# NomaDamas/AutoRAG-Research

Measured on AMD Instinct MI355X. Metric: queries/sec, higher is better.
Workload: dtype f32

## Files before the change

### autorag_research_amd/csrc/dev_common.h

```cpp
#pragma once
#include <hip/hip_runtime.h>
#include <stdint.h>

namespace mi355 {

constexpr int kWave = 64;
constexpr int kQBlockMax = 1024;
constexpr int kKMax = 1024;
constexpr int kCandCap = 2048;
constexpr int kCandCapWide = 4096;
constexpr int kSortMax = 4096;
constexpr int kIrrCap = 1024;
constexpr uint64_t kKeyNaN = 0xFFFFFFFFFFFFFFFFull;

constexpr int kStOverflow = 1;
constexpr int kStIrregular = 2;

struct QueryState {
    float* qn;
    uint16_t* qhat;
    float* thr;
    int* cnt;
    int* best_n;
    uint64_t* best_key;
// ... 362 lines not shown
                    stage_commit(tile, p2, lane);
                    if (k0 + 5 * kStageCols < d) issue(p2, k0 + 5 * kStageCols);
                    acc = chain_piece(tile, lane, qv + k0 + 2 * kStageCols, min(kStageCols, d - k0 - 2 * kStageCols), acc);
                }
            }
        }
    } else {
        for (int k0 = 0; k0 < d; k0 += kStageCols) {
            stage_rows(tile, my_row, k0, d, lane);
            acc = chain_piece(tile, lane, qv + k0, min(kStageCols, d - k0), acc);
        }
    }
    return acc;
}

__device__ __forceinline__ float chain_piece16(const float* tile, int lane, const float* qv, int kn_words, float acc) {
    const float* t = tile + lane * kStageLd;
    for (int w = 0; w + 4 <= kn_words; w += 4) {
        const uint4 tv = *(const uint4*)(t + w);
        const float4 qa = *(const float4*)(qv + 2 * w), qb = *(const float4*)(qv + 2 * w + 4);
        acc = __builtin_fmaf(__uint_as_float(tv.x << 16), qa.x, acc);
        acc = __builtin_fmaf(__uint_as_float(tv.x & 0xFFFF0000u), qa.y, acc);
        acc = __builtin_fmaf(__uint_as_float(tv.y << 16), qa.z, acc);
        acc = __builtin_fmaf(__uint_as_float(tv.y & 0xFFFF0000u), qa.w, acc);
        acc = __builtin_fmaf(__uint_as_float(tv.z << 16), qb.x, acc);
        acc = __builtin_fmaf(__uint_as_float(tv.z & 0xFFFF0000u), qb.y, acc);
        acc = __builtin_fmaf(__uint_as_float(tv.w << 16), qb.z, acc);
        acc = __builtin_fmaf(__uint_as_float(tv.w & 0xFFFF0000u), qb.w, acc);
    }
    return acc;
// ... 23 lines not shown
```

### autorag_research_amd/csrc/index.h

```cpp
#pragma once
#include <climits>
#include <hip/hip_runtime.h>

#include <algorithm>
#include <cmath>
#include <cstdio>
#include <cstring>
#include <mutex>
#include <string>
#include <vector>

#include "dev_common.h"
#include "mi355dr.h"

namespace mi355 {
struct EventPair {
    hipEvent_t a, b;
    int big;
};
struct MultiVecStore;
struct Pending {
    bool active = false;
    hipEvent_t done = nullptr;
    int* status_host = nullptr;
// ... 48 lines not shown

    int path = 0;
    int screen_dtype = 0;
    int retry_level = 0;
    int i8_backoff = 0, i8_probation = 0;
    int i8_demoted_k = INT_MAX;
    double i8_min_budget = 0.25;
    float* retry_q[3] = {nullptr, nullptr, nullptr};
    double* retry_dist[3] = {nullptr, nullptr, nullptr};
    int64_t* retry_rows[3] = {nullptr, nullptr, nullptr};
    int* retry_map[3] = {nullptr, nullptr, nullptr};
    mi355::Pending pend[mi355::kPendingRing];
    mi355::Pending sub_pend[4];
    int64_t seq_next = 0, seq_done = 0;
    int k_now = 10;
    int maxsim_coop = -1;
    int maxsim_persistent = 0;
    int maxsim_wg = -1;
    int maxsim_tighten = 1;
    int maxsim_aligned = 1;
    int maxsim_wg_min = 8;
    int maxsim_wg_pipe = 1;
    int maxsim_pack8 = -1;
    int maxsim_wg_bps = 4;
    int maxsim_pass_groups = 4;
    int maxsim_screen = 1;
    int64_t row_offset = 0;
    int round_a = 0;
    int screen_rq = 1;
    int screen_stream = 1;
    int prefilter16 = 0;
    int profile = 0;
    int starter = 1;
    int prune_companion = 1;
    int scan_dma = 1;
    int defer_round_b = 1;
    int chunk0_set = 0;
    int64_t chunk0_rows = 1024;
    int64_t chunk_growth = 3;
    int chunk_growth_set = 0;
    int64_t small_chunk_rows = 16384;
    int cap = mi355::kCandCap;
    int cap_set = 0;
    int prune_wide = 1;
    int screen_flush_sync = 1, screen_flush_lanes = 48, screen_flush_alone = 40;
    int wide_inflation_x10 = 100;
    int flush_mask_now = -1;
    int chunk_taper_x100 = 0;
    int64_t starter_rows_wide = 65536;

    int64_t s_screen_launches = 0, s_screen_ns = 0, s_screen_rows = 0, s_fallback_queries = 0, s_chunks = 0,
            s_passes = 0, s_candidates = 0, s_rescored = 0, s_starters = 0;
    int64_t s_big_launches = 0, s_big_ns = 0, s_big_rows = 0;
    int screen_rq_split_tests = 1;
    int64_t debug_park = 0;
    float* park_thr = nullptr;
    int screen_drift = 3;
    int* rq_progress = nullptr;
    int rq_epoch = 0;
// ... 63 lines not shown
```

### autorag_research_amd/csrc/k_prune_wide.h

```cpp
#pragma once
#include <type_traits>

#include "k_select.h"

namespace mi355 {

constexpr int kWideEntries = 4096;
constexpr int kWideKeep = 512;
constexpr int kWideList = 1024;
constexpr int kWideKMin = 33, kWideKMax = 128;
constexpr int kWideSortWhole = 256;

__host__ __device__ inline size_t prune_wide_lds_bytes(int d, int waves) {
    return (size_t)kWideKeep * 12 + (size_t)waves * kStageFloats * sizeof(float) + (size_t)kWideList * 4 +
           prune_qs_floats(d) * 4;
}

__device__ __forceinline__ float f32_from_order_key(uint32_t k) {
    return __uint_as_float((k & 0x80000000u) ? (k & 0x7FFFFFFFu) : ~k);
}

template <int WAVES, int PER>
__global__ __launch_bounds__(WAVES * kWave) void k_prune_wide(PruneArgs a) {
    constexpr int T = WAVES * kWave;
    static_assert(T * PER == kWideEntries && (PER == 32 || PER == 64), "entries");
    typedef std::conditional_t<PER == 64, unsigned long long, uint32_t> amask_t;
    constexpr int KS = kWideKeep / T;
    extern __shared__ __attribute__((aligned(16))) char smem[];
    uint64_t* SK = (uint64_t*)smem;
    int32_t* SR = (int32_t*)(smem + (size_t)kWideKeep * 8);
    float* tiles = (float*)(smem + (size_t)kWideKeep * 12);
    uint64_t* K2 = (uint64_t*)tiles;
    int32_t* R2 = (int32_t*)((char*)tiles + (size_t)kWideKeep * 8);
    int32_t* RL = (int32_t*)((char*)tiles + (size_t)WAVES * kStageFloats * sizeof(float));
    float* qs = (float*)((char*)RL + (size_t)kWideList * 4);
    int* scal = (int*)(qs + prune_qs_floats(a.d) - 16);
    const int q = a.qlist ? a.qlist[blockIdx.x] : blockIdx.x;
    const int tid = threadIdx.x;
    const int lane = tid & 63;
    const int wave = __builtin_amdgcn_readfirstlane(tid >> 6);
    const int raw_cnt = a.st.cnt[q];
    const int n_best = a.st.best_n[q];
    if (raw_cnt == 0) return;
    if (raw_cnt > a.cap || raw_cnt > kWideEntries) {
        if (tid == 0) {
            a.st.status[q] |= kStOverflow;
            a.st.cnt[q] = 0;
            a.st.carry[q] = 0;
        }
        return;
    }
    const int n_new = raw_cnt;
    const int32_t* crow = a.cand_row + (int64_t)q * a.cap;
    const float* cval = a.cand_val + (int64_t)q * a.cap;
    uint64_t* bkey = a.st.best_key + (int64_t)q * kKMax;
    int32_t* brow = a.st.best_row + (int64_t)q * kKMax;
    const float nq = a.st.qn[q];
    const float inv_qn = 1.0f / sqrtf(nq);
    const float E = a.st.E[q];
    if (tid == 0) {
        a.stat[2 * q] += (unsigned long long)(n_new - a.st.carry[q]);
        scal[4] = 0;
    }

    int par = 0;
    auto wg_sum = [&](int v) __attribute__((always_inline)) -> int {
        if constexpr (WAVES == 1) return v;
        if (lane == 0) scal[par * WAVES + wave] = v;
        __syncthreads();
        int c = 0;
#pragma unroll
        for (int w = 0; w < WAVES; ++w) c += scal[par * WAVES + w];
        par ^= 1;
        return __builtin_amdgcn_readfirstlane(c);
    };
    auto wg_scan = [&](int v, int& before) __attribute__((always_inline)) -> int {
        if constexpr (WAVES == 1) {
// ... 6 lines not shown
#pragma unroll
        for (int w = 0; w < WAVES; ++w) {
            const int x = scal[par * WAVES + w];
            c += x;
            if (w < wave) b += x;
        }
        par ^= 1;
        before = __builtin_amdgcn_readfirstlane(b);
        return __builtin_amdgcn_readfirstlane(c);
    };
    auto mbcnt = [&](unsigned long long bal) __attribute__((always_inline)) -> int {
        return (int)__builtin_amdgcn_mbcnt_hi((unsigned)(bal >> 32), __builtin_amdgcn_mbcnt_lo((unsigned)bal, 0));
    };

    uint32_t key[PER];
    int32_t rowv[PER];
    amask_t in_a = 0;
    load_candidate_keys<PER, T, true>(key, cval, crow, a.flag8, n_new, tid, rowv);
    for (int k = tid; k < a.d; k += T) qs[k] = a.q[(int64_t)q * a.d + k];
    auto count_ge = [&](uint32_t x) __attribute__((always_inline)) -> int {
        int c = 0;
#pragma unroll
        for (int j = 0; j < PER; ++j) {
            if (j * T >= n_new) break;
            c += __builtin_popcountll(__builtin_amdgcn_ballot_w64(key[j] >= x));
        }
        return wg_sum(c);
    };
    const int n_cand = count_ge(1u);

    auto list_rows = [&](auto&& want, int off, int room, bool mark) __attribute__((always_inline)) -> int {
        int c = 0;
#pragma unroll
        for (int j = 0; j < PER; ++j) {
            if (j * T >= n_new) break;
            c += __builtin_popcountll(__builtin_amdgcn_ballot_w64(want(j)));
        }
        int n = 0;
        const int tot = wg_scan(c, n);
#pragma unroll
        for (int j = 0; j < PER; ++j) {
            if (j * T >= n_new) break;
            const bool w = want(j);
            const unsigned long long bal = __builtin_amdgcn_ballot_w64(w);
            const int pos = n + mbcnt(bal) - off;
            if (w && pos >= 0 && pos < room) {
                RL[pos] = rowv[j];
                if (mark) in_a |= (amask_t)1 << j;
            }
            n += __builtin_popcountll(bal);
        }
        return tot;
    };

    float* tile = tiles + (size_t)wave * kStageFloats;
    auto exact_kth_image = [&](uint32_t (&sk)[KS], int n, int kth, bool with_nan) __attribute__((always_inline)) -> uint32_t {
#pragma unroll
        for (int j = 0; j < KS; ++j) {
            const int e = j * T + tid;
            uint32_t kk = 0;
            if (e < n) {
                const uint64_t k64 = SK[e];
                if (k64 != kKeyNaN) kk = f32_order_key(sim_of_dist(a.metric, key_to_dist(k64)));
                else if (with_nan) kk = 1u;
            }
            sk[j] = kk;
        }
        uint32_t x = 0;
        for (int b = 31; b >= 0; --b) {
            const uint32_t t = x | (1u << b);
// ... 36 lines not shown
            for (int i = tid; i < n; i += T) {
                K2[i] = SK[i];
                R2[i] = SR[i];
            }
        }
        const int np = next_pow2(max(n_sel, 1));
        for (int i = n_sel + tid; i < np; i += T) {
            K2[i] = kKeyNaN;
            R2[i] = 0x7FFFFFFF;
        }
        __syncthreads();
        bitonic_asc_key_row(K2, R2, np);
        return n_sel;
    };

    const int wantA = min(n_cand, min(2 * kWave, max(a.k, a.round_a > 0 ? a.round_a : max(32, 2 * a.k))));
    int nA = 0;
    if (wantA > 0) {
        uint32_t x = 0;
        for (int b = 31; b >= 12; --b) {
            const uint32_t t = x | (1u << b);
            if (count_ge(t) >= wantA) x = t;
        }
        if (x == 0) x = 1u;
        constexpr int kAMax = 2 * kWave;
        nA = min(kAMax, list_rows([&](int j) { return key[j] >= x; }, 0, kAMax, true));
        __syncthreads();
        for (int base = 0; base < nA; base += T) {
            const int e = base + tid;
            const bool live = e < nA;
            const int32_t row = live ? RL[e] : -1;
            const float* rp = live ? a.rows + (int64_t)row * a.d : nullptr;
            if (base + wave * kWave < nA) {
                const float acc = staged_dot(tile, rp, qs, a.d, lane);
                if (live) {
                    SK[n_best + e] = dist_to_key(distance_from(a.metric, acc, nq, a.nrm2[row]));
                    SR[n_best + e] = row;
                }
            }
        }
    }
    for (int i = tid; i < n_best; i += T) {
        SK[i] = bkey[i];
        SR[i] = brow[i];
    }
    __syncthreads();
    const int n1 = n_best + nA;
    int n_sel = select_sort(n1);
    int carried = 0, nB_rescored = 0;
    if (n_cand > nA && !a.thr_only) {
        float cut = -__builtin_inff();
        uint32_t keep_x = 0;
        if (n1 >= a.k && K2[a.k - 1] != kKeyNaN) {
            const float kth = sim_of_dist(a.metric, key_to_dist(K2[a.k - 1]));
            const float ku = a.metric == 0 ? kth : kth * inv_qn;
            cut = ku - fabsf(ku) * (a.metric == 0 ? 0.0f : 4e-6f) - E * 1.001f - 2e-6f * a.cscale;
            keep_x = f32_order_key(kth);
        }
        const uint32_t xB = cut == -__builtin_inff() ? 1u : f32_order_key(cut);
        auto wantB = [&](int j) { return key[j] >= xB && key[j] != 0 && !((in_a >> j) & (amask_t)1); };
        if (a.defer_b && cut != -__builtin_inff()) {
            int32_t* crow_w = a.cand_row + (int64_t)q * a.cap;
            float* cval_w = a.cand_val + (int64_t)q * a.cap;
            int c = 0;
#pragma unroll
            for (int j = 0; j < PER; ++j) {
                if (j * T >= n_new) break;
                c += __builtin_popcountll(__builtin_amdgcn_ballot_w64(wantB(j)));
            }
            int pos0 = 0;
            carried = wg_scan(c, pos0);
#pragma unroll
            for (int j = 0; j < PER; ++j) {
                if (j * T >= n_new) break;
                const bool w = wantB(j);
                const unsigned long long bal = __builtin_amdgcn_ballot_w64(w);
                const int pos = pos0 + mbcnt(bal);
                if (w) {
                    crow_w[pos] = rowv[j];
                    cval_w[pos] = f32_from_order_key(key[j]);
                }
                pos0 += __builtin_popcountll(bal);
            }
        } else {
            const int n_keepA = min(a.k, n_sel);
            for (int i = tid; i < n_keepA; i += T) {
                SK[i] = K2[i];
                SR[i] = R2[i];
            }
            if (tid == 0) scal[4] = n_keepA;
            int totB = 0;
            for (int off = 0; off == 0 || off < totB; off += kWideList) {
                totB = list_rows(wantB, off, kWideList, false);
                __syncthreads();
                const int m = min(kWideList, totB - off);
                for (int base = 0; base < m; base += T) {
                    const int e = base + tid;
                    const bool live = e < m;
                    const int32_t row = live ? RL[e] : -1;
                    const float* rp = live ? a.rows + (int64_t)row * a.d : nullptr;
                    if (base + wave * kWave < m) {
                        const float acc = staged_dot(tile, rp, qs, a.d, lane);
                        uint64_t k64 = kKeyNaN;
                        bool pass = false;
                        if (live) {
                            k64 = dist_to_key(distance_from(a.metric, acc, nq, a.nrm2[row]));
                            pass = keep_x == 0 ||
                                   (k64 != kKeyNaN && f32_order_key(sim_of_dist(a.metric, key_to_dist(k64))) >= keep_x);
                        }
                        const unsigned long long bal = __builtin_amdgcn_ballot_w64(pass);
                        int at = 0;
                        if (lane == 0 && bal != 0) at = atomicAdd(&scal[4], __builtin_popcountll(bal));
                        at = __shfl(at, 0, kWave) + mbcnt(bal);
                        if (pass) {
                            SK[at] = k64;
                            SR[at] = row;
                        }
                    }
                    __syncthreads();
                    const int fill = __builtin_amdgcn_readfirstlane(scal[4]);
                    if (fill + T > kWideKeep) {
                        const int ns = select_sort(fill);
                        const int nk = min(a.k, ns);
                        for (int i = tid; i < nk; i += T) {
                            SK[i] = K2[i];
                            SR[i] = R2[i];
                        }
                        if (nk >= a.k && K2[a.k - 1] != kKeyNaN)
                            keep_x = max(keep_x, f32_order_key(sim_of_dist(a.metric, key_to_dist(K2[a.k - 1]))));
                        __syncthreads();
                        if (tid == 0) scal[4] = nk;
                        __syncthreads();
                    }
                }
                nB_rescored += m;
            }
            n_sel = select_sort(__builtin_amdgcn_readfirstlane(scal[4]));
        }
    }
    if (tid == 0) a.stat[2 * q + 1] += (unsigned long long)(nA + nB_rescored);
    const int n_keep = min(a.k, n_sel);
    if (!a.thr_only)
        for (int i = tid; i < n_keep; i += T) {
            bkey[i] = K2[i];
            brow[i] = R2[i];
        }
    if (tid == 0) {
        if (!a.thr_only) a.st.best_n[q] = n_keep;
        a.st.cnt[q] = carried;
        a.st.carry[q] = carried;
        if (n_keep >= a.k) {
            const uint64_t wk = K2[a.k - 1];
// ... 11 lines not shown
```

### autorag_research_amd/csrc/k_select.h

```cpp
#pragma once
#include "dev_common.h"

namespace mi355 {

struct PruneArgs {
    const float* rows;
    const float* nrm2;
    const float* q;
    QueryState st;
    int32_t* cand_row;
    float* cand_val;
    const int* qlist;
    unsigned long long* stat;
    int cap, d, k, metric;
    int exact;
    const uint8_t* flag8;
    float cscale;
    const uint16_t* shadow16;
    int dpad;
    int round_a;
    int* skip_list;
    int skip_parity;
    int thr_only;
    int one_wave_only;
    int defer_b;
};

__device__ __forceinline__ float unit_sim(int metric, double dist, float inv_qn) {
    return metric == 0 ? (float)(1.0 - dist) : (float)(-dist) * inv_qn;
}
__device__ __forceinline__ float screen_threshold(int metric, double dist_k, float E, float nq) {
    if (metric == 0) return float_below((float)((1.0 - dist_k) - (double)E));
    const double u = -dist_k / sqrt((double)nq);
    return float_below((float)(u - fabs(u) * 4e-6 - (double)E));
}

constexpr int kPruneSmallThreads = 64, kPruneSmallSort = 1024;
constexpr int kPruneBigThreads = 256, kPruneBigSort = kSortMax;

__host__ __device__ inline size_t prune_qs_floats(int d) { return ((size_t)d + 3) / 4 * 4 + 16; }
__host__ __device__ inline size_t prune_lds_bytes(int d, int threads, int sortmax, int dpad16) {
    size_t x = (size_t)(threads / kWave) * kStageFloats * sizeof(float);
    size_t lf = (size_t)sortmax * sizeof(float);
    if (lf > x) x = lf;
    return (size_t)sortmax * 8 + (size_t)sortmax * 4 + x + (size_t)sortmax * 4 + prune_qs_floats(d) * 4 + (size_t)dpad16 * 4;
}

template <int PER, int T, bool ROWS = false>
__device__ __forceinline__ void load_candidate_keys(uint32_t (&key)[PER], const float* __restrict__ cval,
                                                    const int32_t* __restrict__ crow, const uint8_t* __restrict__ flag8,
                                                    int n_new, int tid, int32_t* rows_out = nullptr) {
    float v[PER];
    int32_t r[PER];
// ... 96 lines not shown
            a.skip_list[2 + a.skip_parity * kQBlockMax + i] = q;
        }
    };
    if (raw_cnt > a.cap) {
        if (SORT < kPruneBigSort) {
            leave_for_general();
            return;
        }
        if (tid == 0) {
            a.st.status[q] |= kStOverflow;
            a.st.cnt[q] = 0;
        }
        return;
    }
    if (n_best + raw_cnt > SORT) {
        if (SORT < kPruneBigSort) leave_for_general();
        return;
    }
    const int n_new = raw_cnt;
    const int32_t* crow = a.cand_row + (int64_t)q * a.cap;
    const float* cval = a.cand_val + (int64_t)q * a.cap;
    uint64_t* bkey = a.st.best_key + (int64_t)q * kKMax;
    int32_t* brow = a.st.best_row + (int64_t)q * kKMax;
    const float nq = a.st.qn[q];
    const float inv_qn = 1.0f / sqrtf(nq);
    const float E = a.st.E[q];
    if (tid == 0) {
        a.stat[2 * q] += (unsigned long long)(n_new - a.st.carry[q]);
        a.st.carry[q] = 0;
    }

// ... 416 lines not shown
```

### autorag_research_amd/csrc/mi355dr.hip

```cpp
#include "index.h"
#include "k_prep.h"
#include "k_scan.h"
#include "k_screen.h"
#include "k_screen256c.h"
#include "k_screen_rq.h"

#define MI355_RQ_FORMS(X) X(1) X(2) X(3) X(4) X(5) X(6)
inline bool screen_rq_has(int ksteps) { return ksteps >= 1 && ksteps <= 6; }
#include "k_screen_stream.h"
#include "k_select.h"
#include "k_prune_wide.h"

using namespace mi355;

namespace {
std::mutex g_err_mu;
std::string g_err;
}

namespace mi355 {
int fail(mi355dr_index* idx, int code, const std::string& msg) {
    if (idx) idx->err = msg;
    else {
        std::lock_guard<std::mutex> g(g_err_mu);
// ... 93 lines not shown
    HIPCHECK(idx, hipMalloc(&idx->out_dist_dev, B * kKMax * sizeof(double)));
    HIPCHECK(idx, hipMalloc(&idx->out_rows_dev, B * kKMax * sizeof(int64_t)));
    HIPCHECK(idx, hipMalloc(&idx->prune_skip, (2 + 2 * B) * sizeof(int)));
    HIPCHECK(idx, hipMalloc(&idx->stat_dev, 2 * B * sizeof(unsigned long long)));
    HIPCHECK(idx, hipMemsetAsync(idx->stat_dev, 0, 2 * B * sizeof(unsigned long long), idx->stream));
    if (prune_lds_bytes(idx->dim, kPruneBigThreads, kPruneBigSort, 0) > 160 * 1024 || scan_lds_bytes(idx->dim, 1) > 160 * 1024)
        return fail(idx, MI355DR_E_UNSUPPORTED, "dim too large for the select kernels' LDS budget");
    HIPCHECK(idx, hipFuncSetAttribute((const void*)k_prune<kPruneBigThreads, kPruneBigSort>,
                                      hipFuncAttributeMaxDynamicSharedMemorySize,
                                      (int)prune_lds_bytes(idx->dim, kPruneBigThreads, kPruneBigSort, 0)));
    HIPCHECK(idx, hipFuncSetAttribute((const void*)k_prune<kPruneSmallThreads, kPruneSmallSort>,
                                      hipFuncAttributeMaxDynamicSharedMemorySize,
                                      (int)prune_lds_bytes(idx->dim, kPruneSmallThreads, kPruneSmallSort, idx->dpad)));
    HIPCHECK(idx, hipFuncSetAttribute((const void*)k_prune_wide<2, 32>, hipFuncAttributeMaxDynamicSharedMemorySize,
                                      (int)prune_wide_lds_bytes(idx->dim, 2)));
    {
        int per = kScanQ;
        while (per > 1 && scan_lds_bytes(idx->dim, per) > 150 * 1024) per >>= 1;
        HIPCHECK(idx, hipFuncSetAttribute((const void*)k_scan, hipFuncAttributeMaxDynamicSharedMemorySize,
                                          (int)scan_lds_bytes(idx->dim, per)));
    }
    HIPCHECK(idx, hipFuncSetAttribute((const void*)k_scan32, hipFuncAttributeMaxDynamicSharedMemorySize, kScan32Lds));
    HIPCHECK(idx, hipFuncSetAttribute((const void*)k_screen<false>, hipFuncAttributeMaxDynamicSharedMemorySize, kScreenLds));
    HIPCHECK(idx, hipFuncSetAttribute((const void*)k_screen<true>, hipFuncAttributeMaxDynamicSharedMemorySize, kScreenLds));
    {
        const int stream_lds = kStreamQueryBytesMax + kStreamStages * kStreamStageBytes;
        HIPCHECK(idx, hipFuncSetAttribute((const void*)k_screen_stream<false, 32>, hipFuncAttributeMaxDynamicSharedMemorySize, stream_lds));
        HIPCHECK(idx, hipFuncSetAttribute((const void*)k_screen_stream<true, 32>, hipFuncAttributeMaxDynamicSharedMemorySize, stream_lds));
        HIPCHECK(idx, hipFuncSetAttribute((const void*)k_screen_stream<false, 64>, hipFuncAttributeMaxDynamicSharedMemorySize, stream_lds));
        HIPCHECK(idx, hipFuncSetAttribute((const void*)k_screen_stream<true, 64>, hipFuncAttributeMaxDynamicSharedMemorySize, stream_lds));
// ... 39 lines not shown
        float ms = 0.f;
        if (hipEventElapsedTime(&ms, p.a, p.b) == hipSuccess) {
            idx->s_screen_ns += (int64_t)(ms * 1e6);
            if (p.big) idx->s_big_ns += (int64_t)(ms * 1e6);
        }
        idx->ev_pool.push_back(p);
    }
    idx->ev_pending.swap(keep);
}

constexpr double kInflationBf16 = 5.0, kInflationI8 = 16.0;
constexpr double kSmallBlockBudget = 1.6;
constexpr double kInflationI8Wide = 10.0, kInflationBf16Wide = 4.0;
inline bool wide_ok(const mi355dr_index* idx, int k) { return idx->prune_wide && k >= kWideKMin && k <= kWideKMax; }
inline bool wide_now(const mi355dr_index* idx) { return wide_ok(idx, idx->k_now) && idx->path != MI355DR_PATH_SCAN; }
inline int cap_now(const mi355dr_index* idx) { return !idx->cap_set && wide_now(idx) ? kCandCapWide : idx->cap; }
inline double growth_budget(const mi355dr_index* idx, int k, bool i8) {
    if (wide_ok(idx, k) && idx->path != MI355DR_PATH_SCAN) {
        const int room = std::min(kWideEntries, idx->cap_set ? idx->cap : kCandCapWide);
        return 0.75 * room / ((double)k * (i8 ? idx->wide_inflation_x10 / 10.0 : kInflationBf16Wide)) - 1.0;
    }
    const int room = k < kPruneSmallSort / 2 ? kPruneSmallSort - k : idx->cap;
    return 0.6 * std::min(room, idx->cap) / ((double)k * (i8 ? kInflationI8 : kInflationBf16));
}

inline bool i8_available(const mi355dr_index* idx) { return idx->irr8_n <= kIrrCap; }
inline bool use_i8(const mi355dr_index* idx) {
    if (idx->retry_level > 0) return false;
    if (idx->screen_dtype == MI355DR_SCREEN_I8) return true;
    return idx->screen_dtype == MI355DR_SCREEN_AUTO && i8_available(idx) && idx->k_now < idx->i8_demoted_k &&
           growth_budget(idx, idx->k_now, true) >= idx->i8_min_budget;
}

int launch_prune(mi355dr_index* idx, hipStream_t s, int nblocks, const int* qlist, int k, int exact, bool thr_only = false,
                 bool one_wave_only = false, bool defer_b = false) {
    PruneArgs pa{};
    pa.thr_only = thr_only ? 1 : 0;
    pa.one_wave_only = one_wave_only ? 1 : 0;
    pa.defer_b = defer_b && idx->defer_round_b ? 1 : 0;
    pa.rows = idx->rows;
    pa.nrm2 = idx->nrm2;
    pa.q = idx->qdev;
    pa.st = idx->st;
    pa.cand_row = idx->cand_row;
    pa.cand_val = idx->cand_val;
    pa.qlist = qlist;
    pa.stat = idx->stat_dev;
    pa.cap = cap_now(idx);
    pa.d = idx->dim;
    pa.k = k;
    pa.metric = idx->metric;
    pa.exact = exact;
    pa.flag8 = (use_i8(idx) && idx->irr8_n > 0) ? idx->flag8 : nullptr;
    pa.cscale = idx->metric == MI355DR_METRIC_IP ? idx->cmax : 1.0f;
    pa.shadow16 = (use_i8(idx) && idx->metric == 0 && !exact && idx->prefilter16) ? idx->shadow : nullptr;
    pa.dpad = idx->dpad;
    pa.round_a = idx->round_a;
    if (!exact && wide_now(idx)) {
        pa.shadow16 = nullptr;
        hipLaunchKernelGGL((k_prune_wide<2, 32>), dim3(nblocks), dim3(2 * kWave), prune_wide_lds_bytes(idx->dim, 2), s, pa);
        HIPCHECK(idx, hipGetLastError());
        return MI355DR_OK;
    }
    const bool list_mode = qlist == nullptr;
    pa.skip_list = list_mode ? idx->prune_skip : nullptr;
    pa.skip_parity = list_mode ? (idx->prune_parity ^= 1) : 0;
    hipLaunchKernelGGL((k_prune<kPruneSmallThreads, kPruneSmallSort>), dim3(nblocks), dim3(kPruneSmallThreads),
                       prune_lds_bytes(idx->dim, kPruneSmallThreads, kPruneSmallSort, pa.shadow16 ? idx->dpad : 0), s, pa);
    HIPCHECK(idx, hipGetLastError());
    if (one_wave_only) return MI355DR_OK;
    hipLaunchKernelGGL((k_prune<kPruneBigThreads, kPruneBigSort>), dim3(list_mode ? std::min(nblocks, 64) : nblocks),
                       dim3(kPruneBigThreads), prune_lds_bytes(idx->dim, kPruneBigThreads, kPruneBigSort, 0), s, pa);
    HIPCHECK(idx, hipGetLastError());
    return MI355DR_OK;
}
// ... 146 lines not shown
            const int64_t len = end - prev;
            if (len >= 2 * round_rows) end = std::min<int64_t>(n, prev + (len + round_rows / 2) / round_rows * round_rows);
        }
        if (end <= prev) continue;
        p.ends.push_back(end);
        prev = end;
        if (end >= n) break;
    }
    if (p.ends.empty() || p.ends.back() < n) p.ends.push_back(n);
    return p;
}

inline int starter_count(const PassPlan& p) { return (int)((p.sample + kSlabRows - 1) / kSlabRows); }

PassPlan make_plan(const mi355dr_index* idx, int B, int k) {
    double growth = std::max(0.25, std::min((double)idx->chunk_growth, growth_budget(idx, k, use_i8(idx))));
    if (B <= 64 && idx->retry_level == 0 && idx->chunk_growth_set == 0)
        growth = std::max(growth, std::min(8.0, growth_budget(idx, k, use_i8(idx)) * kSmallBlockBudget));
    if (idx->retry_level == 1) growth = std::max(0.25, growth * 0.5);
    if (idx->retry_level >= 2) growth = 0.25;
    return plan_pass(idx, B, k, growth);
}

int run_screen(mi355dr_index* idx, hipStream_t s, int B, int k, const PassPlan& plan) {
    int64_t kept_all_below = 0;
    const bool i8 = use_i8(idx);
    const int side_n = i8 ? idx->irr8_n : idx->irr_n;
    constexpr int kSideMerge = 32;
    bool side_done = false;
    const bool lean = plan.sample > 0 && idx->prune_companion == 0;
    auto timed = [&](bool big, int64_t rows, auto&& launch) -> int {
// ... 66 lines not shown
    st.thr_key[q] = kKeyNaN;
    st.thr_row[q] = 0x7FFFFFFF;
    st.status[q] &= ~kStOverflow;
}

int scan_range(mi355dr_index* idx, hipStream_t s, int off, int nq, int k, int64_t r0, int64_t r1) {
    ScanArgs sa{};
    sa.rows = idx->rows;
    sa.nrm2 = idx->nrm2;
    sa.q = idx->qdev;
    sa.st = idx->st;
    sa.cand_row = idx->cand_row;
    sa.cand_val = idx->cand_val;
    sa.qlist = idx->qlist_dev + off;
    sa.nq = nq;
    sa.cap = cap_now(idx);
    sa.d = idx->dim;
    sa.metric = idx->metric;
    sa.row0 = r0;
    sa.row1 = r1;
    const int64_t grid = (r1 - r0 + kScanThreads - 1) / kScanThreads;
    if (idx->dim % kScan32PieceCols == 0 && idx->scan_dma)
        hipLaunchKernelGGL(k_scan32, dim3((unsigned)grid), dim3(kScanThreads), kScan32Lds, s, sa, idx->n);
    else
        hipLaunchKernelGGL(k_scan, dim3((unsigned)grid), dim3(kScanThreads), scan_lds_bytes(idx->dim, nq), s, sa);
    HIPCHECK(idx, hipGetLastError());
    return launch_prune(idx, s, nq, idx->qlist_dev + off, k, 1);
}

int run_scan(mi355dr_index* idx, hipStream_t s, const std::vector<int>& qs, int k) {
    if (qs.empty()) return MI355DR_OK;
    HIPCHECK(idx, hipMemcpyAsync(idx->qlist_dev, qs.data(), qs.size() * sizeof(int), hipMemcpyHostToDevice, s));
    const int nq_all = (int)qs.size();
    hipLaunchKernelGGL(k_reset_queries, dim3((nq_all + 255) / 256), dim3(256), 0, s, idx->st, idx->qlist_dev, nq_all);
    HIPCHECK(idx, hipGetLastError());
    const int per = kScanQ;
    for (int off = 0; off < nq_all; off += per) {
        const int nq = std::min(per, nq_all - off);
        int64_t done = 0;
        const int cap = cap_now(idx);
        int64_t chunk = std::min<int64_t>(idx->chunk0_rows, cap);
        while (done < idx->n) {
            const int64_t end = std::min<int64_t>(idx->n, done + chunk);
            CHECK(scan_range(idx, s, off, nq, k, done, end));
            if (end - done > cap) {
                HIPCHECK(idx, hipMemcpyAsync(idx->status_host, idx->st.status, kQBlockMax * sizeof(int),
                                             hipMemcpyDeviceToHost, s));
                HIPCHECK(idx, hipStreamSynchronize(s));
                std::vector<int> redo;
                for (int j = 0; j < nq; ++j)
                    if (idx->status_host[qs[off + j]] & kStOverflow) redo.push_back(qs[off + j]);
                if (!redo.empty()) {
                    const int roff = kQBlockMax;
                    HIPCHECK(idx, hipMemcpyAsync(idx->qlist_dev + roff, redo.data(), redo.size() * sizeof(int),
                                                 hipMemcpyHostToDevice, s));
// ... 24 lines not shown
        orow[(int64_t)map[j] * k + i] = sr[(int64_t)j * k + i];
    }
}

int pending_alloc(mi355dr_index* idx, Pending& p) {
    if (!p.status_host) HIPCHECK(idx, hipHostMalloc(&p.status_host, (kQBlockMax + 1) * sizeof(int)));
    if (!p.done) HIPCHECK(idx, hipEventCreateWithFlags(&p.done, hipEventDisableTiming));
    return MI355DR_OK;
}

int enqueue_block(mi355dr_index* idx, hipStream_t s, const float* q_dev, int B, int k, double* out_dist_dev,
                  int64_t* out_rows_dev, Pending& p) {
    CHECK(ensure_qstate(idx));
    CHECK(pending_alloc(idx, p));
    idx->k_now = k;
    if (idx->retry_level == 0 && idx->screen_dtype == MI355DR_SCREEN_AUTO && k >= idx->i8_demoted_k && --idx->i8_probation <= 0)
        idx->i8_demoted_k = INT_MAX;
    const int Bpad = (int)round_up(B, screen_tile(B));
    if (idx->screen_dtype == MI355DR_SCREEN_I8 && !i8_available(idx) && idx->path != MI355DR_PATH_SCAN)
        return fail(idx, MI355DR_E_UNSUPPORTED, "int8 screen unavailable: too many rows outside the residual limit");
    const bool screen_possible = use_i8(idx) ? i8_available(idx) : idx->irr_n <= kIrrCap;
    const bool use_screen = idx->n > 0 && screen_possible && idx->path != MI355DR_PATH_SCAN;
    if (idx->path == MI355DR_PATH_SCREEN && !screen_possible && idx->n > 0)
        return fail(idx, MI355DR_E_UNSUPPORTED, "screen path unavailable (metric or too many irregular rows)");
    if (q_dev != idx->qdev)
        HIPCHECK(idx, hipMemcpyAsync(idx->qdev, q_dev, (size_t)B * idx->dim * sizeof(float), hipMemcpyDeviceToDevice, s));
    PassPlan plan;
    if (use_screen) plan = make_plan(idx, B, k);
    CHECK(launch_prep(idx, s, B, Bpad, idx->metric, starter_count(plan)));
    if (idx->n > 0) {
// ... 495 lines not shown
        idx->screen_drift = (int)value;
    } else if (k == "small_chunk_rows") {
        if (value < 0) return fail(idx, MI355DR_E_INVALID, "small_chunk_rows must be >= 0");
        idx->small_chunk_rows = value;
    } else if (k == "round_a") {
        if (value < 0 || value > 64) return fail(idx, MI355DR_E_INVALID, "round_a must be in [0,64]");
        idx->round_a = (int)value;
    } else if (k == "prefilter16") {
        idx->prefilter16 = value != 0;
    } else if (k == "cand_cap") {
        if (value < 16 || value > kCandCap) return fail(idx, MI355DR_E_INVALID, "cand_cap must be in [16,2048]");
        idx->cap = (int)value;
        idx->cap_set = 1;
    } else if (k == "prune_wide") {
        idx->prune_wide = value != 0;
    } else if (k == "screen_flush_sync") {
        idx->screen_flush_sync = value != 0;
    } else if (k == "screen_flush_lanes") {
        if (value < 1 || value > 64) return fail(idx, MI355DR_E_INVALID, "screen_flush_lanes must be in [1, 64]");
        idx->screen_flush_lanes = (int)value;
    } else if (k == "screen_flush_alone") {
        if (value < 8 || value > 60) return fail(idx, MI355DR_E_INVALID, "screen_flush_alone must be in [8, 60]");
        idx->screen_flush_alone = (int)value;
    } else if (k == "wide_inflation_x10") {
        if (value < 20 || value > 400) return fail(idx, MI355DR_E_INVALID, "wide_inflation_x10 must be in [20, 400]");
        idx->wide_inflation_x10 = (int)value;
    } else if (k == "chunk_taper_x100") {
        if (value != 0 && (value < 100 || value > 300)) return fail(idx, MI355DR_E_INVALID, "chunk_taper_x100 must be 0 (auto) or in [100, 300]");
        idx->chunk_taper_x100 = (int)value;
    } else if (k == "starter_rows_wide") {
// ... 239 lines not shown
```

Baseline: 161,800.

## Add narrow four-wave prune kernel for small k with larger candidate cap

Adds a four-wave variant of the wide prune kernel for k up to 32 and query blocks larger than 64. It uses a 16-row staged dot product that spreads each row's load across four lane groups, keeps row ids in memory rather than registers, and allows higher occupancy. Plans in this mode get a larger candidate cap and a higher chunk growth so fewer screening passes are needed. The cost is more complex code and shifts in register, LDS and occupancy balance. It also changes overflow handling in the general prune path.

After: 161,700, median of 6. About the same (-0.1%).

```diff
diff --git a/autorag_research_amd/csrc/dev_common.h b/autorag_research_amd/csrc/dev_common.h
--- a/autorag_research_amd/csrc/dev_common.h
+++ b/autorag_research_amd/csrc/dev_common.h
@@ -400,6 +400,103 @@
     return acc;
 }
 
+constexpr int kNarrowRows = 16;
+constexpr int kNarrowFloats = kNarrowRows * kStageLd;
+struct StagePieceN {
+    float4 v[4];
+};
+__device__ __forceinline__ float chain_piece_narrow(const float* t, const float* qv, int kn, float acc) {
+    if (kn == kStageCols) {
+#pragma unroll
+        for (int h = 0; h < 8; ++h) {
+            float4 tv[2], q4[2];
+#pragma unroll
+            for (int i = 0; i < 2; ++i) {
+                tv[i] = *(const float4*)(t + 8 * h + 4 * i);
+                q4[i] = *(const float4*)(qv + 8 * h + 4 * i);
+            }
+#pragma unroll
+            for (int i = 0; i < 2; ++i) {
+                acc = __builtin_fmaf(tv[i].x, q4[i].x, acc);
+                acc = __builtin_fmaf(tv[i].y, q4[i].y, acc);
+                acc = __builtin_fmaf(tv[i].z, q4[i].z, acc);
+                acc = __builtin_fmaf(tv[i].w, q4[i].w, acc);
+            }
+        }
+        return acc;
+    }
+    for (int k = 0; k < kn; ++k) acc = __builtin_fmaf(t[k], qv[k], acc);
+    return acc;
+}
+__device__ __forceinline__ float staged_dot_narrow(float* tile, const float* my_row, const float* qv, int d, int lane) {
+    const float* t = tile + (lane & (kNarrowRows - 1)) * kStageLd;
+    const float* own = lane < kNarrowRows ? my_row : nullptr;
+    float acc = 0.0f;
+    if ((d & 3) == 0) {
+        const unsigned long long live = __builtin_amdgcn_ballot_w64(own != nullptr);
+        if (live == 0) return 0.0f;
+        const int sub = lane >> 4, c4 = (lane & 15) * 4;
+        const int src = __builtin_ctzll(live);
+        unsigned long long a = (unsigned long long)own;
+        unsigned plo = (unsigned)(a & 0xFFFFFFFFull), phi = (unsigned)(a >> 32);
+        const unsigned flo = __shfl(plo, src, kWave), fhi = __shfl(phi, src, kWave);
+        if (own == nullptr) {
+            plo = flo;
+            phi = fhi;
+        }
+        const float* r[4];
+#pragma unroll
+        for (int g = 0; g < 4; ++g) {
+            const unsigned lo = __shfl(plo, g * 4 + sub, kWave), hi = __shfl(phi, g * 4 + sub, kWave);
+            r[g] = (const float*)(((unsigned long long)hi << 32) | lo);
+        }
+        auto issue = [&](StagePieceN& p, int k0) __attribute__((always_inline)) {
+            if (k0 + kStageCols <= d) {
+#pragma unroll
+                for (int g = 0; g < 4; ++g) p.v[g] = load_gmem_f4(r[g] + k0 + c4);
+            } else {
+#pragma unroll
+                for (int g = 0; g < 4; ++g) p.v[g] = k0 + c4 < d ? load_gmem_f4(r[g] + k0 + c4) : make_float4(0.f, 0.f, 0.f, 0.f);
+            }
+        };
+        auto commit = [&](const StagePieceN& p) __attribute__((always_inline)) {
+            wave_sync();
+#pragma unroll
+            for (int g = 0; g < 4; ++g) *(float4*)(tile + (g * 4 + sub) * kStageLd + c4) = p.v[g];
+            wave_sync();
+        };
+        StagePieceN p0, p1;
+        issue(p0, 0);
+        if (kStageCols < d) issue(p1, kStageCols);
+        for (int k0 = 0; k0 < d; k0 += 2 * kStageCols) {
+            commit(p0);
+            if (k0 + 2 * kStageCols < d) issue(p0, k0 + 2 * kStageCols);
+            acc = chain_piece_narrow(t, qv + k0, min(kStageCols, d - k0), acc);
+            if (k0 + kStageCols < d) {
+                commit(p1);
+                if (k0 + 3 * kStageCols < d) issue(p1, k0 + 3 * kStageCols);
+                acc = chain_piece_narrow(t, qv + k0 + kStageCols, min(kStageCols, d - k0 - kStageCols), acc);
+            }
+        }
+        return acc;
+    }
+    const unsigned long long a = (unsigned long long)own;
+    const unsigned plo = (unsigned)(a & 0xFFFFFFFFull), phi = (unsigned)(a >> 32);
+    for (int k0 = 0; k0 < d; k0 += kStageCols) {
+        wave_sync();
+#pragma unroll 4
+        for (int s = 0; s < kNarrowRows; ++s) {
+            const unsigned lo = __shfl(plo, s, kWave), hi = __shfl(phi, s, kWave);
+            const float* rr = (const float*)(((unsigned long long)hi << 32) | lo);
+            const int k = k0 + lane;
+            tile[s * kStageLd + lane] = (rr != nullptr && k < d) ? rr[k] : 0.0f;
+        }
+        wave_sync();
+        acc = chain_piece_narrow(t, qv + k0, min(kStageCols, d - k0), acc);
+    }
+    return acc;
+}
+
 __device__ __forceinline__ float chain_piece16(const float* tile, int lane, const float* qv, int kn_words, float acc) {
     const float* t = tile + lane * kStageLd;
     for (int w = 0; w + 4 <= kn_words; w += 4) {
diff --git a/autorag_research_amd/csrc/index.h b/autorag_research_amd/csrc/index.h
--- a/autorag_research_amd/csrc/index.h
+++ b/autorag_research_amd/csrc/index.h
@@ -86,6 +86,7 @@
     mi355::Pending sub_pend[4];
     int64_t seq_next = 0, seq_done = 0;
     int k_now = 10;
+    int b_now = mi355::kQBlockMax;
     int maxsim_coop = -1;
     int maxsim_persistent = 0;
     int maxsim_wg = -1;
@@ -115,6 +116,8 @@
     int cap = mi355::kCandCap;
     int cap_set = 0;
     int prune_wide = 1;
+    int prune_mw = 1;
+    int64_t mw_growth = 7;
     int screen_flush_sync = 1, screen_flush_lanes = 48, screen_flush_alone = 40;
     int wide_inflation_x10 = 100;
     int flush_mask_now = -1;
diff --git a/autorag_research_amd/csrc/k_prune_wide.h b/autorag_research_amd/csrc/k_prune_wide.h
--- a/autorag_research_amd/csrc/k_prune_wide.h
+++ b/autorag_research_amd/csrc/k_prune_wide.h
@@ -10,29 +10,38 @@
 constexpr int kWideList = 1024;
 constexpr int kWideKMin = 33, kWideKMax = 128;
 constexpr int kWideSortWhole = 256;
-
-__host__ __device__ inline size_t prune_wide_lds_bytes(int d, int waves) {
-    return (size_t)kWideKeep * 12 + (size_t)waves * kStageFloats * sizeof(float) + (size_t)kWideList * 4 +
-           prune_qs_floats(d) * 4;
+constexpr int kMwKMax = 32;
+
+__host__ __device__ constexpr size_t prune_wide_tile_bytes(int waves, bool narrow) {
+    return (size_t)waves * (narrow ? kNarrowFloats : kStageFloats) * sizeof(float) > (size_t)kWideKeep * 12
+               ? (size_t)waves * (narrow ? kNarrowFloats : kStageFloats) * sizeof(float)
+               : (size_t)kWideKeep * 12;
+}
+__host__ __device__ inline size_t prune_wide_lds_bytes(int d, int waves, bool narrow = false) {
+    return (size_t)kWideKeep * 12 + prune_wide_tile_bytes(waves, narrow) + (size_t)kWideList * 4 + prune_qs_floats(d) * 4;
 }
 
 __device__ __forceinline__ float f32_from_order_key(uint32_t k) {
     return __uint_as_float((k & 0x80000000u) ? (k & 0x7FFFFFFFu) : ~k);
 }
 
-template <int WAVES, int PER>
-__global__ __launch_bounds__(WAVES * kWave) void k_prune_wide(PruneArgs a) {
+template <int WAVES, int PER, bool NARROW = false>
+__global__ __launch_bounds__(WAVES * kWave, NARROW ? 4 : 1) void k_prune_wide(PruneArgs a) {
     constexpr int T = WAVES * kWave;
-    static_assert(T * PER == kWideEntries && (PER == 32 || PER == 64), "entries");
+    static_assert(T * PER == kWideEntries && (PER == 16 || PER == 32 || PER == 64), "entries");
+    static_assert(!NARROW || WAVES == 4, "the narrow gather is the four-wave form's");
     typedef std::conditional_t<PER == 64, unsigned long long, uint32_t> amask_t;
     constexpr int KS = kWideKeep / T;
+    constexpr int RW = NARROW ? kNarrowRows : kWave;
+    constexpr int kBatch = WAVES * RW;
+    constexpr int kFill = 2 * WAVES;
     extern __shared__ __attribute__((aligned(16))) char smem[];
     uint64_t* SK = (uint64_t*)smem;
     int32_t* SR = (int32_t*)(smem + (size_t)kWideKeep * 8);
     float* tiles = (float*)(smem + (size_t)kWideKeep * 12);
     uint64_t* K2 = (uint64_t*)tiles;
     int32_t* R2 = (int32_t*)((char*)tiles + (size_t)kWideKeep * 8);
-    int32_t* RL = (int32_t*)((char*)tiles + (size_t)WAVES * kStageFloats * sizeof(float));
+    int32_t* RL = (int32_t*)((char*)tiles + prune_wide_tile_bytes(WAVES, NARROW));
     float* qs = (float*)((char*)RL + (size_t)kWideList * 4);
     int* scal = (int*)(qs + prune_qs_floats(a.d) - 16);
     const int q = a.qlist ? a.qlist[blockIdx.x] : blockIdx.x;
@@ -60,7 +69,7 @@
     const float E = a.st.E[q];
     if (tid == 0) {
         a.stat[2 * q] += (unsigned long long)(n_new - a.st.carry[q]);
-        scal[4] = 0;
+        scal[kFill] = 0;
     }
 
     int par = 0;
@@ -97,9 +106,10 @@
     };
 
     uint32_t key[PER];
-    int32_t rowv[PER];
+    constexpr bool kRowsInRegs = !NARROW;
+    int32_t rowv[kRowsInRegs ? PER : 1];
     amask_t in_a = 0;
-    load_candidate_keys<PER, T, true>(key, cval, crow, a.flag8, n_new, tid, rowv);
+    load_candidate_keys<PER, T, kRowsInRegs>(key, cval, crow, a.flag8, n_new, tid, rowv);
     for (int k = tid; k < a.d; k += T) qs[k] = a.q[(int64_t)q * a.d + k];
     auto count_ge = [&](uint32_t x) __attribute__((always_inline)) -> int {
         int c = 0;
@@ -113,6 +123,8 @@
     const int n_cand = count_ge(1u);
 
     auto list_rows = [&](auto&& want, int off, int room, bool mark) __attribute__((always_inline)) -> int {
+        int tid_e = tid;
+        if constexpr (!kRowsInRegs) asm volatile("" : "+v"(tid_e));
         int c = 0;
 #pragma unroll
         for (int j = 0; j < PER; ++j) {
@@ -128,7 +140,8 @@
             const unsigned long long bal = __builtin_amdgcn_ballot_w64(w);
             const int pos = n + mbcnt(bal) - off;
             if (w && pos >= 0 && pos < room) {
-                RL[pos] = rowv[j];
+                if constexpr (kRowsInRegs) RL[pos] = rowv[j];
+                else RL[pos] = j * T + tid_e;
                 if (mark) in_a |= (amask_t)1 << j;
             }
             n += __builtin_popcountll(bal);
@@ -136,7 +149,19 @@
         return tot;
     };
 
-    float* tile = tiles + (size_t)wave * kStageFloats;
+    float* tile = tiles + (size_t)wave * (NARROW ? kNarrowFloats : kStageFloats);
+    auto gather = [&](int base, int rpw, int m, auto&& store) __attribute__((always_inline)) {
+        const int e = base + wave * rpw + lane;
+        const bool live = lane < rpw && e < m;
+        const int32_t row = live ? (kRowsInRegs ? RL[e] : crow[RL[e]]) : -1;
+        const float* rp = live ? a.rows + (int64_t)row * a.d : nullptr;
+        if (base + wave * rpw < m) {
+            float acc;
+            if constexpr (NARROW) acc = staged_dot_narrow(tile, rp, qs, a.d, lane);
+            else acc = staged_dot(tile, rp, qs, a.d, lane);
+            store(live, e, row, acc);
+        }
+    };
     auto exact_kth_image = [&](uint32_t (&sk)[KS], int n, int kth, bool with_nan) __attribute__((always_inline)) -> uint32_t {
 #pragma unroll
         for (int j = 0; j < KS; ++j) {
@@ -203,7 +228,8 @@
         return n_sel;
     };
 
-    const int wantA = min(n_cand, min(2 * kWave, max(a.k, a.round_a > 0 ? a.round_a : max(32, 2 * a.k))));
+    constexpr int kAMax = NARROW ? kBatch : 2 * kWave;
+    const int wantA = min(n_cand, min(kAMax, max(a.k, a.round_a > 0 ? a.round_a : max(32, 2 * a.k))));
     int nA = 0;
     if (wantA > 0) {
         uint32_t x = 0;
@@ -212,22 +238,16 @@
             if (count_ge(t) >= wantA) x = t;
         }
         if (x == 0) x = 1u;
-        constexpr int kAMax = 2 * kWave;
         nA = min(kAMax, list_rows([&](int j) { return key[j] >= x; }, 0, kAMax, true));
         __syncthreads();
-        for (int base = 0; base < nA; base += T) {
-            const int e = base + tid;
-            const bool live = e < nA;
-            const int32_t row = live ? RL[e] : -1;
-            const float* rp = live ? a.rows + (int64_t)row * a.d : nullptr;
-            if (base + wave * kWave < nA) {
-                const float acc = staged_dot(tile, rp, qs, a.d, lane);
+        const int rpw = NARROW ? (nA + WAVES - 1) / WAVES : kWave;
+        for (int base = 0; base < nA; base += WAVES * rpw)
+            gather(base, rpw, nA, [&](bool live, int e, int32_t row, float acc) __attribute__((always_inline)) {
                 if (live) {
                     SK[n_best + e] = dist_to_key(distance_from(a.metric, acc, nq, a.nrm2[row]));
                     SR[n_best + e] = row;
                 }
-            }
-        }
+            });
     }
     for (int i = tid; i < n_best; i += T) {
         SK[i] = bkey[i];
@@ -251,6 +271,17 @@
         if (a.defer_b && cut != -__builtin_inff()) {
             int32_t* crow_w = a.cand_row + (int64_t)q * a.cap;
             float* cval_w = a.cand_val + (int64_t)q * a.cap;
+            int32_t crv[kRowsInRegs ? 1 : PER];
+            if constexpr (!kRowsInRegs) {
+                int tid_e = tid;
+                asm volatile("" : "+v"(tid_e));
+#pragma unroll
+                for (int j = 0; j < PER; ++j) {
+                    if (j * T >= n_new) break;
+                    if (wantB(j)) crv[j] = crow[j * T + tid_e];
+                }
+                asm volatile("s_waitcnt vmcnt(0)" ::: "memory");
+            }
             int c = 0;
 #pragma unroll
             for (int j = 0; j < PER; ++j) {
@@ -266,7 +297,8 @@
                 const unsigned long long bal = __builtin_amdgcn_ballot_w64(w);
                 const int pos = pos0 + mbcnt(bal);
                 if (w) {
-                    crow_w[pos] = rowv[j];
+                    if constexpr (kRowsInRegs) crow_w[pos] = rowv[j];
+                    else crow_w[pos] = crv[j];
                     cval_w[pos] = f32_from_order_key(key[j]);
                 }
                 pos0 += __builtin_popcountll(bal);
@@ -277,19 +309,15 @@
                 SK[i] = K2[i];
                 SR[i] = R2[i];
             }
-            if (tid == 0) scal[4] = n_keepA;
+            if (tid == 0) scal[kFill] = n_keepA;
             int totB = 0;
             for (int off = 0; off == 0 || off < totB; off += kWideList) {
                 totB = list_rows(wantB, off, kWideList, false);
                 __syncthreads();
                 const int m = min(kWideList, totB - off);
-                for (int base = 0; base < m; base += T) {
-                    const int e = base + tid;
-                    const bool live = e < m;
-                    const int32_t row = live ? RL[e] : -1;
-                    const float* rp = live ? a.rows + (int64_t)row * a.d : nullptr;
-                    if (base + wave * kWave < m) {
-                        const float acc = staged_dot(tile, rp, qs, a.d, lane);
+                for (int base = 0, rpw = RW; base < m; base += WAVES * rpw) {
+                    if (NARROW) rpw = min(RW, (m - base + WAVES - 1) / WAVES);
+                    gather(base, rpw, m, [&](bool live, int e, int32_t row, float acc) __attribute__((always_inline)) {
                         uint64_t k64 = kKeyNaN;
                         bool pass = false;
                         if (live) {
@@ -299,16 +327,16 @@
                         }
                         const unsigned long long bal = __builtin_amdgcn_ballot_w64(pass);
                         int at = 0;
-                        if (lane == 0 && bal != 0) at = atomicAdd(&scal[4], __builtin_popcountll(bal));
+                        if (lane == 0 && bal != 0) at = atomicAdd(&scal[kFill], __builtin_popcountll(bal));
                         at = __shfl(at, 0, kWave) + mbcnt(bal);
                         if (pass) {
                             SK[at] = k64;
                             SR[at] = row;
                         }
-                    }
+                    });
                     __syncthreads();
-                    const int fill = __builtin_amdgcn_readfirstlane(scal[4]);
-                    if (fill + T > kWideKeep) {
+                    const int fill = __builtin_amdgcn_readfirstlane(scal[kFill]);
+                    if (fill + kBatch > kWideKeep) {
                         const int ns = select_sort(fill);
                         const int nk = min(a.k, ns);
                         for (int i = tid; i < nk; i += T) {
@@ -318,13 +346,13 @@
                         if (nk >= a.k && K2[a.k - 1] != kKeyNaN)
                             keep_x = max(keep_x, f32_order_key(sim_of_dist(a.metric, key_to_dist(K2[a.k - 1]))));
                         __syncthreads();
-                        if (tid == 0) scal[4] = nk;
+                        if (tid == 0) scal[kFill] = nk;
                         __syncthreads();
                     }
                 }
                 nB_rescored += m;
             }
-            n_sel = select_sort(__builtin_amdgcn_readfirstlane(scal[4]));
+            n_sel = select_sort(__builtin_amdgcn_readfirstlane(scal[kFill]));
         }
     }
     if (tid == 0) a.stat[2 * q + 1] += (unsigned long long)(nA + nB_rescored);
diff --git a/autorag_research_amd/csrc/k_select.h b/autorag_research_amd/csrc/k_select.h
--- a/autorag_research_amd/csrc/k_select.h
+++ b/autorag_research_amd/csrc/k_select.h
@@ -37,6 +37,7 @@
 
 constexpr int kPruneSmallThreads = 64, kPruneSmallSort = 1024;
 constexpr int kPruneBigThreads = 256, kPruneBigSort = kSortMax;
+static_assert(kSortMax >= kKMax + kCandCap, "the general form sorts a full kept list and a full default candidate list");
 
 __host__ __device__ inline size_t prune_qs_floats(int d) { return ((size_t)d + 3) / 4 * 4 + 16; }
 __host__ __device__ inline size_t prune_lds_bytes(int d, int threads, int sortmax, int dpad16) {
@@ -163,7 +164,15 @@
         return;
     }
     if (n_best + raw_cnt > SORT) {
-        if (SORT < kPruneBigSort) leave_for_general();
+        if (SORT < kPruneBigSort) {
+            leave_for_general();
+            return;
+        }
+        if (tid == 0) {
+            a.st.status[q] |= kStOverflow;
+            a.st.cnt[q] = 0;
+            a.st.carry[q] = 0;
+        }
         return;
     }
     const int n_new = raw_cnt;
diff --git a/autorag_research_amd/csrc/mi355dr.hip b/autorag_research_amd/csrc/mi355dr.hip
--- a/autorag_research_amd/csrc/mi355dr.hip
+++ b/autorag_research_amd/csrc/mi355dr.hip
@@ -131,6 +131,8 @@
                                       (int)prune_lds_bytes(idx->dim, kPruneSmallThreads, kPruneSmallSort, idx->dpad)));
     HIPCHECK(idx, hipFuncSetAttribute((const void*)k_prune_wide<2, 32>, hipFuncAttributeMaxDynamicSharedMemorySize,
                                       (int)prune_wide_lds_bytes(idx->dim, 2)));
+    HIPCHECK(idx, hipFuncSetAttribute((const void*)k_prune_wide<4, 16, true>, hipFuncAttributeMaxDynamicSharedMemorySize,
+                                      (int)prune_wide_lds_bytes(idx->dim, 4, true)));
     {
         int per = kScanQ;
         while (per > 1 && scan_lds_bytes(idx->dim, per) > 150 * 1024) per >>= 1;
@@ -200,11 +202,17 @@
 constexpr double kInflationI8Wide = 10.0, kInflationBf16Wide = 4.0;
 inline bool wide_ok(const mi355dr_index* idx, int k) { return idx->prune_wide && k >= kWideKMin && k <= kWideKMax; }
 inline bool wide_now(const mi355dr_index* idx) { return wide_ok(idx, idx->k_now) && idx->path != MI355DR_PATH_SCAN; }
-inline int cap_now(const mi355dr_index* idx) { return !idx->cap_set && wide_now(idx) ? kCandCapWide : idx->cap; }
+inline bool mw_ok(const mi355dr_index* idx, int k) { return idx->prune_mw && k >= 1 && k <= kMwKMax && idx->b_now > 64; }
+inline bool mw_now(const mi355dr_index* idx) { return mw_ok(idx, idx->k_now) && idx->path != MI355DR_PATH_SCAN; }
+inline int cap_now(const mi355dr_index* idx) { return !idx->cap_set && (wide_now(idx) || mw_now(idx)) ? kCandCapWide : idx->cap; }
 inline double growth_budget(const mi355dr_index* idx, int k, bool i8) {
     if (wide_ok(idx, k) && idx->path != MI355DR_PATH_SCAN) {
         const int room = std::min(kWideEntries, idx->cap_set ? idx->cap : kCandCapWide);
         return 0.75 * room / ((double)k * (i8 ? idx->wide_inflation_x10 / 10.0 : kInflationBf16Wide)) - 1.0;
+    }
+    if (mw_ok(idx, k) && idx->path != MI355DR_PATH_SCAN) {
+        const int room = std::min(kWideEntries, idx->cap_set ? idx->cap : kCandCapWide);
+        return 0.75 * room / ((double)k * (i8 ? kInflationI8 : kInflationBf16)) - 1.0;
     }
     const int room = k < kPruneSmallSort / 2 ? kPruneSmallSort - k : idx->cap;
     return 0.6 * std::min(room, idx->cap) / ((double)k * (i8 ? kInflationI8 : kInflationBf16));
@@ -232,7 +240,7 @@
     pa.cand_val = idx->cand_val;
     pa.qlist = qlist;
     pa.stat = idx->stat_dev;
-    pa.cap = cap_now(idx);
+    pa.cap = exact ? idx->cap : cap_now(idx);
     pa.d = idx->dim;
     pa.k = k;
     pa.metric = idx->metric;
@@ -245,6 +253,13 @@
     if (!exact && wide_now(idx)) {
         pa.shadow16 = nullptr;
         hipLaunchKernelGGL((k_prune_wide<2, 32>), dim3(nblocks), dim3(2 * kWave), prune_wide_lds_bytes(idx->dim, 2), s, pa);
+        HIPCHECK(idx, hipGetLastError());
+        return MI355DR_OK;
+    }
+    if (!exact && mw_now(idx)) {
+        pa.shadow16 = nullptr;
+        hipLaunchKernelGGL((k_prune_wide<4, 16, true>), dim3(nblocks), dim3(4 * kWave), prune_wide_lds_bytes(idx->dim, 4, true), s,
+                           pa);
         HIPCHECK(idx, hipGetLastError());
         return MI355DR_OK;
     }
@@ -421,7 +436,8 @@
 inline int starter_count(const PassPlan& p) { return (int)((p.sample + kSlabRows - 1) / kSlabRows); }
 
 PassPlan make_plan(const mi355dr_index* idx, int B, int k) {
-    double growth = std::max(0.25, std::min((double)idx->chunk_growth, growth_budget(idx, k, use_i8(idx))));
+    const double cap_growth = mw_now(idx) && !idx->chunk_growth_set ? (double)idx->mw_growth : (double)idx->chunk_growth;
+    double growth = std::max(0.25, std::min(cap_growth, growth_budget(idx, k, use_i8(idx))));
     if (B <= 64 && idx->retry_level == 0 && idx->chunk_growth_set == 0)
         growth = std::max(growth, std::min(8.0, growth_budget(idx, k, use_i8(idx)) * kSmallBlockBudget));
     if (idx->retry_level == 1) growth = std::max(0.25, growth * 0.5);
@@ -518,7 +534,7 @@
     sa.cand_val = idx->cand_val;
     sa.qlist = idx->qlist_dev + off;
     sa.nq = nq;
-    sa.cap = cap_now(idx);
+    sa.cap = idx->cap;
     sa.d = idx->dim;
     sa.metric = idx->metric;
     sa.row0 = r0;
@@ -542,7 +558,7 @@
     for (int off = 0; off < nq_all; off += per) {
         const int nq = std::min(per, nq_all - off);
         int64_t done = 0;
-        const int cap = cap_now(idx);
+        const int cap = idx->cap;
         int64_t chunk = std::min<int64_t>(idx->chunk0_rows, cap);
         while (done < idx->n) {
             const int64_t end = std::min<int64_t>(idx->n, done + chunk);
@@ -597,6 +613,7 @@
     CHECK(ensure_qstate(idx));
     CHECK(pending_alloc(idx, p));
     idx->k_now = k;
+    idx->b_now = B;
     if (idx->retry_level == 0 && idx->screen_dtype == MI355DR_SCREEN_AUTO && k >= idx->i8_demoted_k && --idx->i8_probation <= 0)
         idx->i8_demoted_k = INT_MAX;
     const int Bpad = (int)round_up(B, screen_tile(B));
@@ -1122,6 +1139,11 @@
         idx->cap_set = 1;
     } else if (k == "prune_wide") {
         idx->prune_wide = value != 0;
+    } else if (k == "prune_mw") {
+        idx->prune_mw = value != 0;
+    } else if (k == "mw_growth") {
+        if (value < 1 || value > 63) return fail(idx, MI355DR_E_INVALID, "mw_growth must be in [1, 63]");
+        idx->mw_growth = value;
     } else if (k == "screen_flush_sync") {
         idx->screen_flush_sync = value != 0;
     } else if (k == "screen_flush_lanes") {
```
